# kevin-robb/live_ekf_slam

Measured on AMD Instinct MI355X. Metric: EKF predict-update steps/sec @ L=50, batch=65536; fp64 state RMSE vs ref, higher is better.
Workload: dtype f64

## Files before the change

live_ekf_slam_amd/csrc/capi_state.cpp:

```cpp
#include <stdio.h>
#include <string.h>

#include <vector>

#include "slam_handle.h"
#include "ekf_kernel.h"
#include "ukf_kernel.h"

using namespace slam_capi;

extern "C" {

int slam_get_sigma_points(slam_handle* h, int inst, double* X, int32_t* rows, int32_t* cols) {
    if (!h || inst < 0 || inst >= h->B) return slam_internal_fail(SLAM_ERR_ARG, "bad instance");
    TRY(flush_lazy(h));
    if (h->kind == SLAM_EKF_SLAM) return slam_internal_fail(SLAM_ERR_UNSUPPORTED, "sigma points exist for the UKF kinds only");
    if (!h->inited) return slam_internal_fail(SLAM_ERR_STATE, "slam_init has not been called");
    HIP_TRY(hipSetDevice(h->device));
    HIP_TRY(hipStreamSynchronize(h->stream));
    int32_t n = 0;
    HIP_TRY(hipMemcpy(&n, h->ukf.dnsq + inst, sizeof(int32_t), hipMemcpyDeviceToHost));
    n = n < 0 ? 0 : (n > h->n_max ? h->n_max : n);
    if (rows) *rows = n;
    if (cols) *cols = n > 0 ? 2 * n + 1 : 0;
// ... 201 lines not shown
    }
    std::vector<char> buf((size_t)64 << 20);
    for (const CkptItem& it : ckpt_items(h))
        for (size_t off = 0; off < it.bytes; off += buf.size()) {
            const size_t nb = it.bytes - off < buf.size() ? it.bytes - off : buf.size();
            if (fread(buf.data(), 1, nb, f) != nb) { fclose(f); return slam_internal_fail(SLAM_ERR_IO, "%s is truncated", path); }
            if (hipMemcpy((char*)it.dev + off, buf.data(), nb, hipMemcpyHostToDevice) != hipSuccess) { fclose(f); return slam_internal_fail(SLAM_ERR_HIP, "copying the state to the device failed"); }
        }
    fclose(f);
    h->step = hd.step; h->inited = hd.inited != 0; h->seed = hd.seed; h->inst0 = hd.inst0;
    h->ukf.predicted = false;
    TRY(map_track_reset(h));
    if (h->shadow) {
        const int tr = h->tracked;
        const int rc = slam_track_instance(h, tr);
        if (rc) return rc;
    }
    return SLAM_OK;
}

int slam_track_instance(slam_handle* h, int inst) {
    if (!h || inst >= h->B) return slam_internal_fail(SLAM_ERR_ARG, "bad instance");
    TRY(flush_lazy(h));
    if (h->ukf.predicted) return slam_internal_fail(SLAM_ERR_STATE, "a prediction stage is pending: call slam_update_dev first");
    if (h->shadow) { slam_destroy(h->shadow); h->shadow = nullptr; h->tracked = -1; }
    if (inst < 0) return SLAM_OK;
    if (h->kind != SLAM_EKF_SLAM) return slam_internal_fail(SLAM_ERR_UNSUPPORTED, "EKF handles only: the UKF launches every step at the call, there is no queue a getter would have to run");
    HIP_TRY(hipSetDevice(h->device));
    HIP_TRY(hipStreamSynchronize(h->stream));
    slam_handle* s = nullptr;
    int rc = slam_create(&h->cfg, h->kind, 1, h->L_max, h->dtype, h->device, &s);
    if (rc) return rc;
    s->lazy_max = 0;
    s->seed = h->seed; s->inst0 = h->inst0 + inst;
    s->range_max = h->range_max; s->fov_min = h->fov_min; s->fov_max = h->fov_max;
    s->waves_per_filter = h->waves_per_filter;
    if (!h->hmap.empty()) rc = slam_set_map(s, h->hmap.data(), (int)(h->hmap.size() / 2));
    if (!rc && h->each.maps_each)
        rc = slam_set_maps(s, h->each.hmaps.data() + (size_t)inst * h->each.map_stride * 2, h->each.hLs.data() + inst, h->each.map_stride);
    if (!rc && h->each.noise_each) rc = slam_set_noise_each(s, h->each.hnoise.data() + inst);
    if (!rc && h->inited) {
        const size_t b = (size_t)inst, e = (size_t)h->esz;
        hipError_t errs[] = {
            hipMemcpy(s->dP, (const char*)h->dP + b * h->pstride * e, (size_t)h->pstride * e, hipMemcpyDeviceToDevice),
            hipMemcpy(s->dx, (const char*)h->dx + b * h->xstride * e, (size_t)h->xstride * e, hipMemcpyDeviceToDevice),
            hipMemcpy(s->dM, h->dM + b, sizeof(int32_t), hipMemcpyDeviceToDevice),
            hipMemcpy(s->dids, h->dids + b * h->L_max, sizeof(int32_t) * h->L_max, hipMemcpyDeviceToDevice),
            hipMemcpy(s->dflags, h->dflags + b, sizeof(int32_t), hipMemcpyDeviceToDevice),
            hipMemcpy(s->dts, h->dts + b, sizeof(int32_t), hipMemcpyDeviceToDevice),
            hipMemcpy(s->dtruth, h->dtruth + 3 * b, sizeof(double) * 3, hipMemcpyDeviceToDevice),
            hipMemcpy(s->derr, h->derr + b, sizeof(double), hipMemcpyDeviceToDevice),
            h->ukf.dsq ? hipMemcpy(s->ukf.dsq, h->ukf.dsq + b * h->pstride, sizeof(double) * h->pstride, hipMemcpyDeviceToDevice) : hipSuccess,
            h->ukf.dnsq ? hipMemcpy(s->ukf.dnsq, h->ukf.dnsq + b, sizeof(int32_t), hipMemcpyDeviceToDevice) : hipSuccess,
            h->ukf.dxprev ? hipMemcpy(s->ukf.dxprev, h->ukf.dxprev + b * h->xstride, sizeof(double) * h->xstride, hipMemcpyDeviceToDevice) : hipSuccess,
            h->ukf.dvt ? hipMemcpy(s->ukf.dvt, h->ukf.dvt + b * h->pstride, sizeof(double) * h->pstride, hipMemcpyDeviceToDevice) : hipSuccess,
            h->ukf.dvage ? hipMemcpy(s->ukf.dvage, h->ukf.dvage + b, sizeof(int32_t), hipMemcpyDeviceToDevice) : hipSuccess,
        };
        for (hipError_t ee : errs)
            if (ee != hipSuccess) { slam_destroy(s); return slam_internal_fail(SLAM_ERR_HIP, "copying the tracked instance -> %s", hipGetErrorString(ee)); }
        s->step = h->step; s->inited = true;
    }
    if (rc) { slam_destroy(s); return rc; }
    h->shadow = s; h->tracked = inst;
    return SLAM_OK;
}

int slam_sync(slam_handle* h) {
    if (!h) return slam_internal_fail(SLAM_ERR_ARG, "NULL handle");
    TRY(flush_lazy(h));
    HIP_TRY(hipSetDevice(h->device));
    HIP_TRY(hipStreamSynchronize(h->stream));
    h->eager_target = h->eager_init;
    return SLAM_OK;
}
int slam_batch(const slam_handle* h) { return h ? h->B : 0; }
int slam_state_dim_max(const slam_handle* h) { return h ? h->n_max : 0; }

int slam_set_debug_flags(slam_handle* h, int flags) {
    if (!h) return slam_internal_fail(SLAM_ERR_ARG, "NULL handle");
    TRY(flush_lazy(h));
    HIP_TRY(hipSetDevice(h->device));
    HIP_TRY(hipStreamSynchronize(h->stream));
#ifndef SLAM_ABLATE
    flags &= (4 | 32 | 128);
#endif
    if ((flags & (4 | 32)) && !h->dprof) {
        HIP_TRY(h->dprof.reserve(slam::kEkfProfSlots * (size_t)h->B));
        HIP_TRY(hipMemset(h->dprof, 0, sizeof(unsigned long long) * h->dprof.cap()));
    }
    h->dbg = flags;
    return SLAM_OK;
}

int slam_variant_available(int L_max, int dtype, int variant) { return slam::ekf_variant_available(L_max, dtype == SLAM_F32, variant); }

int slam_k_histogram(slam_handle* h, uint64_t out[8], int reset) {
    if (!h || !out) return slam_internal_fail(SLAM_ERR_ARG, "bad argument");
    TRY(flush_lazy(h));
    HIP_TRY(hipSetDevice(h->device));
    HIP_TRY(h->kind == SLAM_EKF_SLAM ? hipStreamSynchronize(h->stream) : hipDeviceSynchronize());
    static_assert(sizeof(unsigned long long) == sizeof(uint64_t), "histogram element size");
    HIP_TRY(hipMemcpy(out, h->dkhist, sizeof(uint64_t) * 8, hipMemcpyDeviceToHost));
    if (reset) HIP_TRY(hipMemset(h->dkhist, 0, sizeof(uint64_t) * 8));
    return SLAM_OK;
}

int slam_traffic_counters(slam_handle* h, uint64_t out[4], int reset) {
    if (!h || !out) return slam_internal_fail(SLAM_ERR_ARG, "bad argument");
    if (h->kind != SLAM_EKF_SLAM) return slam_internal_fail(SLAM_ERR_UNSUPPORTED, "the traffic counters are kept by the EKF step kernels");
    TRY(flush_lazy(h));
    HIP_TRY(hipSetDevice(h->device));
    HIP_TRY(hipStreamSynchronize(h->stream));
    HIP_TRY(hipMemcpy(out, h->dkhist + slam::kEkfTrafficSlot, sizeof(uint64_t) * 4, hipMemcpyDeviceToHost));
    if (reset) HIP_TRY(hipMemset(h->dkhist + slam::kEkfTrafficSlot, 0, sizeof(uint64_t) * 4));
    return SLAM_OK;
}

int slam_reset_counters_async(slam_handle* h) {
    if (!h) return slam_internal_fail(SLAM_ERR_ARG, "bad argument");
    TRY(flush_lazy(h));
    HIP_TRY(hipSetDevice(h->device));
    HIP_TRY(hipMemsetAsync(h->dkhist, 0, sizeof(unsigned long long) * 16, h->stream));
    return SLAM_OK;
}

int slam_kernel_info(slam_handle* h, int multi_step, char* name, int name_cap, int32_t out[5]) {
    if (!h || (!name && !out)) return slam_internal_fail(SLAM_ERR_ARG, "bad argument");
    if (h->kind != SLAM_EKF_SLAM) return slam_internal_fail(SLAM_ERR_UNSUPPORTED, "EKF handles only");
    HIP_TRY(hipSetDevice(h->device));
    slam::EkfKernelInfo ki;
    HIP_TRY(slam::ekf_kernel_info(h->L_max, h->B, h->waves_per_filter, h->esz == 4, multi_step ? 1 : 0, &ki));
    if (name && name_cap > 0) { strncpy(name, ki.name, (size_t)name_cap - 1); name[name_cap - 1] = 0; }
    if (out) {
        hipDeviceProp_t pr;
        HIP_TRY(hipGetDeviceProperties(&pr, h->device));
        out[0] = ki.lds_bytes; out[1] = ki.vgprs; out[2] = ki.threads; out[3] = ki.wg_per_cu; out[4] = pr.multiProcessorCount;
    }
    return SLAM_OK;
}

int slam_ukf_sweep_stats(slam_handle* h, uint64_t out[2], int reset) {
    if (!h || !out) return slam_internal_fail(SLAM_ERR_ARG, "bad argument");
    if (h->kind == SLAM_EKF_SLAM) return slam_internal_fail(SLAM_ERR_STATE, "UKF handles only");
    TRY(flush_lazy(h));
    HIP_TRY(hipSetDevice(h->device));
    HIP_TRY(hipDeviceSynchronize());
    HIP_TRY(hipMemcpy(out, h->dkhist + 8, sizeof(uint64_t) * 2, hipMemcpyDeviceToHost));
    if (reset) HIP_TRY(hipMemset(h->dkhist + 8, 0, sizeof(uint64_t) * 2));
    return SLAM_OK;
}

int slam_ukf_set_sqrt_mode(slam_handle* h, int mode) {
    if (!h) return slam_internal_fail(SLAM_ERR_ARG, "bad argument");
    if (h->kind == SLAM_EKF_SLAM) return slam_internal_fail(SLAM_ERR_ARG, "the square-root mode is a UKF setting");
    if (mode != SLAM_UKF_SQRT_EIGEN && mode != SLAM_UKF_SQRT_CHOLESKY) return slam_internal_fail(SLAM_ERR_ARG, "unknown square-root mode %d", mode);
    if (mode == SLAM_UKF_SQRT_CHOLESKY && h->L_max > slam::kUkfLdsMaxLandmarks)
        return slam_internal_fail(SLAM_ERR_UNSUPPORTED, "the Cholesky square root exists for the LDS size classes only (L_max <= %d), this handle has L_max %d",
                                  slam::kUkfLdsMaxLandmarks, h->L_max);
    TRY(flush_lazy(h));
    HIP_TRY(hipSetDevice(h->device));
    if (mode == SLAM_UKF_SQRT_CHOLESKY) HIP_TRY(h->ukf.dchol.reserve((size_t)h->B));
    h->ukf.chol = mode == SLAM_UKF_SQRT_CHOLESKY;
    return SLAM_OK;
}

int slam_ukf_sqrt_stats(slam_handle* h, uint64_t out[2], int reset) {
    if (!h || !out) return slam_internal_fail(SLAM_ERR_ARG, "bad argument");
// ... 63 lines not shown
```

live_ekf_slam_amd/csrc/ekf_kernel_impl.h:

```cpp
#pragma once
#include "ekf_kernel.h"

#include <stdio.h>

#include <type_traits>

#include "../../include/slam_batch.h"
#include "ekf_model.h"
#include "slam_rng.h"
#include "sim_device.h"

namespace slam {

template <int NMAX, int W, int KG_, int UNR_, int KP_ = 0>
struct EkfGeom {
    static constexpr int TPB = 64 * W;
    static constexpr int LDP = (NMAX + 2) & ~1;
    static constexpr int LMAX = (NMAX - 3) / 2;
    static constexpr int KCAP = LMAX > 0 ? LMAX : 1;
    static constexpr int KG = KG_;
    static constexpr int KP = KP_ > 0 ? KP_ : ((KG_ > 5 && NMAX > 43 && W < 5) ? 3 : (KG_ > 4 ? 4 : KG_));
    static constexpr int KLOOP = 2 * KP;
    static constexpr int TS = 3 + 2 * KP;
    static constexpr int UNR = UNR_;
// ... 32 lines not shown
#endif
#ifndef SLAM_CTRL_ILP
#define SLAM_CTRL_ILP 1
#endif
#ifndef SLAM_CTRL_SG
#define SLAM_CTRL_SG 3
#endif
#ifndef SLAM_PRIO_THIN
#define SLAM_PRIO_THIN 2
#endif

#define SLAM_STAMP(i)                                                                    \
    do {                                                                                 \
        if (prof_on && tid == 0) {                                                       \
            const unsigned long long now_ = __builtin_readcyclecounter();                \
            p.prof[(size_t)blockIdx.x * kEkfProfSlots + (i)] += now_ - tprev;                            \
            tprev = now_;                                                                \
        }                                                                                \
    } while (0)

typedef double dbl2_t __attribute__((ext_vector_type(2)));
typedef float flt4_t __attribute__((ext_vector_type(4)));
template <class ST> struct Vec16;
template <> struct Vec16<double> {
    static constexpr int VEC = 2;
    typedef dbl2_t type;
};
template <> struct Vec16<float> {
    static constexpr int VEC = 4;
    typedef flt4_t type;
};

__device__ __forceinline__ int opaque(int v) {
    asm volatile("" : "+v"(v));
    return v;
}

typedef const __attribute__((address_space(4))) EkfStepParams* EkfColdParams;
__device__ __forceinline__ EkfColdParams ekf_cold_params() {
    EkfColdParams k = (EkfColdParams)__builtin_amdgcn_kernarg_segment_ptr();
    asm volatile("" : "+s"(k));
    return k;
}
struct EkfSimCold {
    uint64_t seed;
    int64_t inst0;
    double d_max, th_max, range_max, fov_min, fov_max;
};
struct EkfMapCold {
    const double* map;
    const double* map_each;
    const int32_t* L_each;
    int32_t map_stride, L;
};
struct EkfSimNoiseCold {
    double sV00, sV11, sW00, sW11;
    const NoiseRow* noise_each;
    int32_t sim;
};

__device__ __forceinline__ double rdlane(double v, int l) {
    const int lo = __builtin_amdgcn_readlane(__double2loint(v), l);
    const int hi = __builtin_amdgcn_readlane(__double2hiint(v), l);
    return __hiloint2double(hi, lo);
}

__device__ __forceinline__ unsigned hi_abs(double v) {
    return (unsigned)(__double_as_longlong(v) >> 32) & 0x7fffffffu;
}

template <int NMAX, int W, int KG_, int UNR_, class ST, int PIPE, bool MULTI, int KP_ = 0>
__global__ __launch_bounds__(64 * W, (W >= 2 ? 4 : SLAM_W1_WAVES)) void ekf_step_kernel(const EkfStepParams p) {
    using G = EkfGeom<NMAX, W, KG_, UNR_, KP_>;
    constexpr int TPB = G::TPB, LDP = G::LDP, KCAP = G::KCAP, LMAX = G::LMAX, KG = G::KG, KP = G::KP, KLOOP = G::KLOOP, TS = G::TS, UNR = G::UNR;

    __shared__ double s_xt[LDP];
    __shared__ double s_xp[LDP];
    __shared__ double s_R[TS * LDP];
    __shared__ double s_C[TS * LDP];
    __shared__ double2 s_K[KG * LDP];
    constexpr int VEC = Vec16<ST>::VEC;
    constexpr int HS = hp_substride<VEC>(LDP), HPW = (VEC - 1) * HS + (LDP + VEC - 1) / VEC;
    __shared__ double2 s_HP[KG * HPW];
    __shared__ double s_sc[16];
    constexpr int SD = SLAM_SD;
    __shared__ float s_meas[SD * 3 * KCAP];
    __shared__ double s_tru[SD * 6];
    __shared__ int s_kraw[SD];
    __shared__ int s_sim[2];
    __shared__ int s_ids[LMAX > 0 ? LMAX : 1];
    __shared__ int s_didx[2 * KCAP];
    __shared__ int s_next[2 * 4];
    __shared__ double s_ps[2 * 10];
    __shared__ int s_chunk;
    __shared__ int s_T[TS];
    __shared__ signed char s_slot[LDP];
    __shared__ signed char s_need[TS];
    __shared__ int s_misc[8];
    __shared__ double s_keep[4];
    __shared__ int s_kh[8];
    __shared__ int s_ring[8];
    __shared__ int s_pass[4];
    __shared__ int s_wend[KG];
    __shared__ unsigned s_cnt[4];

    const int b = blockIdx.x;
    const int tid = threadIdx.x;
    const int lane = tid & 63;
    const FilterNoise nz = filter_noise(p, b);
    if (p.long_mode == 1) {
        const int kk = p.meas_count_in[b];
        if ((kk < p.k_stride_in ? kk : p.k_stride_in) > p.long_cap) return;
    }

    const bool dump_meas = p.meas_out != nullptr;
    const bool prof_on = (p.dbg & 4) && p.prof != nullptr;
    unsigned long long tprev = prof_on ? __builtin_readcyclecounter() : 0ull;
    if (prof_on && tid < 64) p.prof[(size_t)blockIdx.x * kEkfProfSlots + tid] = 0ull;
    typedef typename Vec16<ST>::type VT;
    constexpr int ESZ = (int)sizeof(ST);
    auto hpi = [](int c) -> int { return (c & (VEC - 1)) * HS + (c / VEC); };
    const int T = MULTI ? p.T : 1;
    ST* const PA = const_cast<ST*>(static_cast<const ST*>(p.P)) + (size_t)b * p.pstride;
    ST* const PB = static_cast<ST*>(p.P_out) + (size_t)b * p.pstride;
    ST* const Pfinal = PA;
    ST* Pcur = PA;
    ST* __restrict__ xb = static_cast<ST*>(p.x) + (size_t)b * p.xstride;
    constexpr bool kWide = sizeof(ST) == 8;
    int flags = p.flags[b];
    const int M_init = p.M[b];
    double xpre[(LDP + TPB - 1) / TPB];
#pragma unroll
    for (int u = 0; u < (LDP + TPB - 1) / TPB; ++u) {
        const int i = tid + TPB * u;
        xpre[u] = (i < p.xstride && i < LDP) ? (double)xb[i] : 0.0;
    }
    const int idpre = (tid < p.L_max) ? p.ids[(size_t)b * p.L_max + tid] : 0;
    double keep0 = 0.0;
    if (p.sim && tid < 64) {
        if (tid < 3) keep0 = p.truth[3 * (size_t)b + tid];
        if (tid == 3) keep0 = p.err_sum[b];
    }
    const int n_init = 3 + 2 * M_init;
    const int ts0 = p.timestep[b];

    if (flags & SLAM_INST_INDEX_OOR) {
        return;
    }

#pragma unroll
    for (int u = 0; u < (LDP + TPB - 1) / TPB; ++u) {
        const int i = tid + TPB * u;
        if (i < LDP) {
            const double v = i < n_init ? xpre[u] : 0.0;
            s_xt[i] = v;
            s_xp[i] = v;
        }
    }
    if (tid < M_init) s_ids[tid] = idpre;
    if (tid < 4) s_keep[tid] = keep0;
#pragma unroll 1
    for (int i = tid; i < LDP; i += TPB) s_slot[i] = (signed char)(i < 3 ? i : -1);
    if (tid < TS) {
        s_T[tid] = tid < 3 ? tid : -1;
        s_need[tid] = (signed char)(tid < 3 ? 1 : 0);
    }
    if (tid < 8) s_kh[tid] = 0;
// ... 159 lines not shown
```

live_ekf_slam_amd/csrc/ekf_step_control.h:

```cpp

    auto leader_chain = [&](int ii, int si, float r_m, float b_m, double (&H)[8], double& nu0, double& nu1, double (&Si)[4]) -> bool {
        const double* const xl = p.lm_from_pred ? s_xp : s_xt;
        const double dx = xl[ii] - s_xp[0], dy = xl[ii + 1] - s_xp[1];
        const float dist = (float)sqrt(dx * dx + dy * dy);
        const double dd = (double)dist, d2 = (double)(dist * dist);
        const int hl = lane & 7;
        const bool usey = (hl == 1) || (hl == 3) || (hl == 4) || (hl == 6);
        const bool neg = (hl == 0) || (hl == 1) || (hl == 5) || (hl == 6);
        double num = usey ? dy : dx;
        num = neg ? -num : num;
        const double q = num / (hl < 4 ? dd : d2);
        const float angf = (float)rem2pi(det_atan2(dy, dx) - s_xp[2]);
        const float nu0f = r_m - dist - nz.w_r;
        const float nu1f = b_m - angf - nz.w_b;
        nu0 = (double)nu0f; nu1 = (double)nu1f;
#pragma unroll
        for (int j = 0; j < 8; ++j) H[j] = rdlane(q, j);
        const double h00 = H[0], h01 = H[1], h03 = H[2], h04 = H[3], h10 = H[4], h11 = H[5], h12 = -1.0, h13 = H[6], h14 = H[7];
        const int cs = lane < 3 ? lane : (lane == 3 ? ii : ii + 1);
        const double p0 = s_R[cs], p1 = s_R[LDP + cs], p2 = s_R[2 * LDP + cs], pi = s_R[si * LDP + cs], pj = s_R[(si + 1) * LDP + cs];
        const double gx = ((h00 * p0 + h01 * p1) + h03 * pi) + h04 * pj;
        const double gy = (((h10 * p0 + h11 * p1) + h12 * p2) + h13 * pi) + h14 * pj;
        const double g0x = rdlane(gx, 0), g1x = rdlane(gx, 1), g2x = rdlane(gx, 2), gix = rdlane(gx, 3), gjx = rdlane(gx, 4);
        const double g0y = rdlane(gy, 0), g1y = rdlane(gy, 1), g2y = rdlane(gy, 2), giy = rdlane(gy, 3), gjy = rdlane(gy, 4);
// ... 6 lines not shown
        S[3] = S[3] + nz.W11;
        return inv2x2_lu(S, Si);
    };

    auto form_known = [&](const int* didx_g, int k, int l0, int lim, int nsrc, int& l1_out, int& nT_out) -> int {
        const int l1 = (k - l0 < lim) ? k : l0 + lim;
        const int ng = l1 - l0;
        const int idx = (lane < ng) ? didx_g[l0 + lane] : -1;
        const int myii = idx >= 0 ? 3 + 2 * idx : -1;
        const int cur = (lane < KP) ? s_T[3 + 2 * lane] : -1;
        bool dupl = false, has = false, keep = false;
#pragma unroll
        for (int w = 0; w < KP; ++w) {
            const int ii_w = __builtin_amdgcn_readlane(myii, w), cur_w = __builtin_amdgcn_readlane(cur, w);
            dupl = dupl || (w < lane && ii_w == myii);
            has = has || (cur_w >= 0 && cur_w == myii);
            keep = keep || (ii_w >= 0 && ii_w == cur);
        }
        const bool wantv = myii >= 0 && !dupl;
        const bool release = lane < KP && cur >= 0 && !keep;
        if (release) {
            s_slot[cur] = (signed char)-1; s_slot[cur + 1] = (signed char)-1;
            s_T[3 + 2 * lane] = -1; s_T[4 + 2 * lane] = -1;
        }
        const bool freeslot = lane < KP && (cur < 0 || !keep);
        const unsigned long long fmask = __ballot(freeslot);
        const bool needs = wantv && !has;
        const unsigned long long nmask = __ballot(needs);
        const int rank = __popcll(nmask & ((1ull << lane) - 1ull));
        int j = 0;
        {
            unsigned long long fm = fmask;
#pragma unroll
            for (int w = 0; w < KP; ++w) {
                const int lowest = __ffsll((long long)fm) - 1;
                if (w == rank) j = lowest;
                fm &= fm - 1ull;
            }
        }
        bool gath = false;
        if (needs) {
            s_T[3 + 2 * j] = myii; s_T[4 + 2 * j] = myii + 1;
            s_slot[myii] = (signed char)(3 + 2 * j); s_slot[myii + 1] = (signed char)(4 + 2 * j);
            const signed char nd = (signed char)(myii < nsrc ? 1 : 2);
            s_need[3 + 2 * j] = nd; s_need[4 + 2 * j] = nd;
            gath = nd == 1;
        }
        unsigned long long occ = __ballot(lane < KP && cur >= 0 && keep);
        {
            unsigned long long fm = fmask;
            const int ntake = __popcll(nmask);
#pragma unroll
            for (int w = 0; w < KP; ++w) {
                const int lowest = __ffsll((long long)fm) - 1;
                if (w < ntake && lowest >= 0) occ |= 1ull << lowest;
                fm &= fm - 1ull;
            }
        }
        l1_out = l1;
        nT_out = occ ? 5 + 2 * (63 - __clzll((long long)occ)) : 3;
        return __ballot(gath) != 0ull ? 1 : 0;
    };

    auto thin_downdate = [&](int j0, int jstride, int s0, int sstride, int nTd, int nd, const double2* __restrict__ Ku,
                             const double2* __restrict__ HPu) {
        const int* const Ttab = s_T;
#pragma unroll 1
        for (int j = j0; j < nd; j += jstride) {
            const double2 kj = Ku[j], hj = HPu[hpi(j)];
#pragma unroll 2
            for (int sl = s0; sl < nTd; sl += sstride) {
                const int t_s = Ttab[sl];
                if ((unsigned)t_s < (unsigned)nd) {
                    const double2 kt = Ku[t_s], ht = HPu[hpi(t_s)];
                    const int i = sl * LDP + j;
                    s_R[i] = ekf_downdate(s_R[i], kt.x, kt.y, hj.x, hj.y);
                    s_C[i] = ekf_downdate(s_C[i], kj.x, kj.y, ht.x, ht.y);
                }
            }
        }
    };

    constexpr int NU = (LDP + 63) / 64;
    auto thin_downdate_ctl = [&](int nTd, int nd, const double2* __restrict__ Ku, const double2* __restrict__ HPu, const double2 (&kj)[NU],
                                 const double2 (&hj)[NU]) {
        constexpr int SG = SLAM_CTRL_SG;
        int tsv[TS];
#pragma unroll
        for (int sl = 0; sl < TS; ++sl) tsv[sl] = s_T[sl];
#pragma unroll
        for (int s0 = 0; s0 < TS; s0 += SG) {
            if (s0 >= nTd) break;
            double2 kt[SG], ht[SG];
            double rv[SG][NU], cv[SG][NU];
            bool ok[SG];
#pragma unroll
            for (int g = 0; g < SG; ++g) {
                const int sl = s0 + g < TS ? s0 + g : TS - 1;
                const int t_s = tsv[sl];
                ok[g] = s0 + g < nTd && (unsigned)t_s < (unsigned)nd;
                const int tc = ok[g] ? t_s : 0;
                kt[g] = Ku[tc]; ht[g] = HPu[hpi(tc)];
#pragma unroll
                for (int u = 0; u < NU; ++u) {
                    const int j = lane + 64 * u;
                    const int i = sl * LDP + (j < LDP ? j : 0);
                    rv[g][u] = s_R[i]; cv[g][u] = s_C[i];
                }
            }
#pragma unroll
            for (int g = 0; g < SG; ++g) {
                if (!ok[g]) continue;
                const int sl = s0 + g;
#pragma unroll
                for (int u = 0; u < NU; ++u) {
                    const int j = lane + 64 * u;
                    if (j < nd) {
                        const int i = sl * LDP + j;
                        s_R[i] = ekf_downdate(rv[g][u], kt[g].x, kt[g].y, hj[u].x, hj[u].y);
                        s_C[i] = ekf_downdate(cv[g][u], kj[u].x, kj[u].y, ht[g].x, ht[g].y);
                    }
                }
            }
        }
    };
```

live_ekf_slam_amd/csrc/ekf_step_decoupled.h:

```cpp

    if constexpr (MULTI && W >= 2) {
        auto fastable = [&](int tq) -> bool {
            const int* nx = s_next + 4 * (tq & 1);
            constexpr int kStepMax = sizeof(ST) == 8 ? KLOOP : (KLOOP < KG ? KLOOP : KG);
            return nx[0] <= kStepMax && nx[1] == 0 && nx[2] == 0 && nx[3] == 0;
        };
        const bool fast_ok = p.id_known && !dump_meas && fastable(t) &&
                             !SLAM_DBG(p.dbg & (2 | 16 | 64));
        if (fast_ok) {
            const int n = na, ldn = ekf_ld(n, ESZ);
            ST* const Pbuf = Pcur;
            constexpr int kFirstStreamer = 1;
            constexpr int NS = W - kFirstStreamer;
            constexpr bool kGen = W >= 2;
            if (tid == 0) {
                s_ring[0] = nu; s_ring[1] = 0; s_ring[2] = 0; s_ring[3] = 0; s_ring[4] = t; s_ring[5] = 0; s_ring[6] = 0; s_ring[7] = 0;
                s_pass[0] = 0; s_pass[1] = 0; s_pass[2] = 0; s_pass[3] = 0;
            }
            __syncthreads();
            auto ld_i = [](int* q) -> int { return __hip_atomic_load(q, __ATOMIC_RELAXED, __HIP_MEMORY_SCOPE_WORKGROUP); };
            auto st_i = [](int* q, int v) { __hip_atomic_store(q, v, __ATOMIC_RELAXED, __HIP_MEMORY_SCOPE_WORKGROUP); };
            constexpr int kSpinBudget = 1 << 21;
            auto spin_over = [&](int& spins) -> bool {
                spins += 1;
// ... 84 lines not shown
                                        }
                                    }
                                }
#pragma unroll
                                for (int g = 0; g < GB; ++g)
                                    if (g < nb) {
                                        s_R[ss[g] * LDP + j] = j < n ? rv[g] : 0.0;
                                        s_C[ss[g] * LDP + j] = j < n ? cv[g] : 0.0;
                                    }
                            }
#pragma unroll
                            for (int g = 0; g < GB; ++g)
                                if (g < nb && ss[g] >= 3 && lane < 3) {
                                    s_R[ss[g] * LDP + lane] = s_C[lane * LDP + ts[g]];
                                    s_C[ss[g] * LDP + lane] = s_R[lane * LDP + ts[g]];
                                }
                        }
                        if (lane == 0) st_i(&s_ring[6], 0);
                    }
                    if (lane < TS) s_need[lane] = 0;
                    SLAM_STAMP(18);
                    if (l0q == 0) {
                        const double* const ps = s_ps + 10 * pq;
                        const double* const r2o = s_R + 2 * LDP;
                        const double* const c2o = s_C + 2 * LDP;
                        const double fa = ps[3], fb = ps[4];
                        const double p22 = r2o[2];
                        auto predicted = [&](double tv, int r, int cc) -> double {
                            const double f_r = r == 0 ? fa : fb;
                            if (r < 2) tv = tv + f_r * r2o[cc];
                            if (cc < 2) {
                                double a2 = c2o[r];
                                if (r < 2) a2 = a2 + f_r * p22;
                                tv = tv + a2 * (cc == 0 ? fa : fb);
                            }
                            if (r < 2 && cc < 2) tv = tv + ps[5 + 2 * r + cc];
                            if (r == 2 && cc == 2) tv = tv + nz.V11;
                            return tv;
                        };
                        double n_r0 = 0.0, n_r1 = 0.0, n_c0 = 0.0, n_c1 = 0.0, n_22 = 0.0;
                        const int t_s = (lane >= 2 && lane < nTq) ? s_T[lane] : -1;
                        const bool thin_l = (unsigned)t_s < (unsigned)n;
                        if (thin_l) {
                            n_r0 = predicted(s_R[lane * LDP + 0], t_s, 0);
                            n_r1 = predicted(s_R[lane * LDP + 1], t_s, 1);
                            n_c0 = predicted(s_C[lane * LDP + 0], 0, t_s);
                            n_c1 = predicted(s_C[lane * LDP + 1], 1, t_s);
                            if (lane == 2) n_22 = predicted(p22, 2, 2);
                        }
#pragma unroll
                        for (int u = 0; u < (LDP + 63) / 64; ++u) {
                            const int j = lane + 64 * u;
                            if (j >= 2 && j < n) {
                                const double r2 = r2o[j], c2 = c2o[j];
                                s_R[j] = ekf_pred_row(s_R[j], fa, r2);
                                s_R[LDP + j] = ekf_pred_row(s_R[LDP + j], fb, r2);
                                s_C[j] = ekf_pred_col(s_C[j], c2, fa);
                                s_C[LDP + j] = ekf_pred_col(s_C[LDP + j], c2, fb);
                            }
                        }
                        if (lane < 2) {
                            const int j = lane;
                            const double v00 = predicted(s_R[j], 0, j), v10 = predicted(s_R[LDP + j], 1, j);
                            const double w00 = predicted(s_C[j], j, 0), w10 = predicted(s_C[LDP + j], j, 1);
                            s_R[j] = v00; s_R[LDP + j] = v10; s_C[j] = w00; s_C[LDP + j] = w10;
                        }
                        if (thin_l) {
                            s_R[lane * LDP + 0] = n_r0; s_R[lane * LDP + 1] = n_r1;
                            s_C[lane * LDP + 0] = n_c0; s_C[lane * LDP + 1] = n_c1;
                            if (lane == 2) { s_R[2 * LDP + 2] = n_22; s_C[2 * LDP + 2] = n_22; }
                        }
                    }
                    SLAM_STAMP(19);
#pragma unroll 1
                    for (int l = l0q; l < l1q; ++l) {
                        const int idx = didx_q[l];
                        if (idx < 0) continue;
                        const float r_m = meas_q[3 * l + 1], b_m = meas_q[3 * l + 2];
                        const int ii = 3 + 2 * idx;
                        const int si = s_slot[ii];
                        double H[8], Si[4], nu0, nu1;
                        if (!leader_chain(ii, si, r_m, b_m, H, nu0, nu1, Si)) fl_or |= SLAM_INST_S_SINGULAR;
                        SLAM_STAMP(20);
                        for (int sp = 0; pub - ld_i(&s_ring[1]) >= KG && !spin_over(sp);) __builtin_amdgcn_s_sleep(SLAM_SLEEP_RING);
                        if (ld_i(&s_ring[2])) break;
                        SLAM_STAMP(21);
                        const int slot = pub % KG;
                        double2* __restrict__ HPu = s_HP + slot * HPW;
                        double2* __restrict__ Ku = s_K + slot * LDP;
                        double2 kreg[NU], hreg[NU];
#pragma unroll
                        for (int u = 0; u < NU; ++u) { kreg[u] = make_double2(0.0, 0.0); hreg[u] = make_double2(0.0, 0.0); }
                        if (!SLAM_DBG(p.dbg & 512)) {
                            const double h00 = H[0], h01 = H[1], h03 = H[2], h04 = H[3], h10 = H[4], h11 = H[5], h12 = -1.0, h13 = H[6], h14 = H[7];
                            const double* Ri = s_R + si * LDP;
                            const double* Rj = s_R + (si + 1) * LDP;
                            const double* Ci = s_C + si * LDP;
                            const double* Cj = s_C + (si + 1) * LDP;
#pragma unroll
                            for (int u = 0; u < (LDP + 63) / 64; ++u) {
                                const int c = lane + 64 * u;
                                double2 hp = make_double2(0.0, 0.0), kk = make_double2(0.0, 0.0);
                                if (c < n) {
                                    const double p0 = s_R[c], p1 = s_R[LDP + c], p2 = s_R[2 * LDP + c], pi = Ri[c], pj = Rj[c];
                                    hp.x = ((h00 * p0 + h01 * p1) + h03 * pi) + h04 * pj;
                                    hp.y = (((h10 * p0 + h11 * p1) + h12 * p2) + h13 * pi) + h14 * pj;
                                    const double q0 = s_C[c], q1 = s_C[LDP + c], q2 = s_C[2 * LDP + c], qi = Ci[c], qj = Cj[c];
                                    const double phx = ((q0 * h00 + q1 * h01) + qi * h03) + qj * h04;
                                    const double phy = (((q0 * h10 + q1 * h11) + q2 * h12) + qi * h13) + qj * h14;
                                    kk.x = phx * Si[0] + phy * Si[2];
                                    kk.y = phx * Si[1] + phy * Si[3];
                                    double xv = s_xp[c] + (kk.x * nu0 + kk.y * nu1);
                                    if (c == 2) xv = rem2pi(xv);
                                    s_xp[c] = xv;
                                }
                                if (c < LDP) { HPu[hpi(c)] = hp; Ku[c] = kk; }
                                kreg[u] = kk; hreg[u] = hp;
                            }
                        }
                        if (!kWide && lane == 0) s_wend[slot] = (l == lastu) ? 1 : 0;
                        __builtin_amdgcn_fence(__ATOMIC_RELEASE, "workgroup");
                        pub += 1;
                        if (lane == 0) st_i(&s_ring[0], pub);
                        SLAM_STAMP(22);
                        if (!SLAM_DBG(p.dbg & 256)) {
#if SLAM_CTRL_ILP
                            thin_downdate_ctl(nTq, n, Ku, HPu, kreg, hreg);
#else
                            thin_downdate(lane, 64, 0, 1, nTq, n, Ku, HPu);
#endif
                        }
                    }
                    l0q = l1q;
                    } while (l0q < kq && !ld_i(&s_ring[2]));
                    if (ld_i(&s_ring[2])) break;
                    SLAM_STAMP(23);
                    if (p.sim && lane == 0) {
                        const double* tru = s_tru + (tt % SD) * 6 + 3;
                        const double ex = (double)(float)s_xp[0] - tru[0], ey = (double)(float)s_xp[1] - tru[1];
                        s_keep[3] = s_keep[3] + sqrt(ex * ex + ey * ey);
                    }
#pragma unroll 1
                    for (int i = lane; i < n; i += 64) {
                        const ST sv = (ST)s_xp[i];
                        s_xt[i] = (double)sv;
                        s_xp[i] = (double)sv;
                        const unsigned h0 = hi_abs((double)sv);
                        hiacc = hiacc > h0 ? hiacc : h0;
                    }
                    if constexpr (!kWide) {
                        const int nel = nTq * LDP;
#pragma unroll 1
                        for (int i0 = lane; i0 < nel; i0 += 256) {
                            double rv[4], cv[4];
#pragma unroll
                            for (int u = 0; u < 4; ++u) {
                                const int i = i0 + 64 * u < nel ? i0 + 64 * u : i0;
                                rv[u] = s_R[i]; cv[u] = s_C[i];
                            }
#pragma unroll
                            for (int u = 0; u < 4; ++u) {
                                const int i = i0 + 64 * u;
                                if (i < nel) { s_R[i] = (double)(ST)rv[u]; s_C[i] = (double)(ST)cv[u]; }
                            }
                        }
                    }
                    if ((p.dbg & 32) && p.prof != nullptr && lane == 0 && tt < kEkfProfSlots)
                        p.prof[(size_t)blockIdx.x * kEkfProfSlots + tt] = (wall_clock64() << 4) | (unsigned long long)(kq < 15 ? kq : 15);
                    tt += 1;
                    SLAM_STAMP(24);
                    if (tt >= T) break;
                    if constexpr (kGen) {
                        for (int sp = 0; ld_i(&s_sim[0]) <= tt && !spin_over(sp);) __builtin_amdgcn_s_sleep(1);
                        __builtin_amdgcn_fence(__ATOMIC_ACQUIRE, "workgroup");
                    }
                    SLAM_STAMP(26);
                    prestep(tt);
                    SLAM_STAMP(25);
                    if (!fastable(tt)) break;
                }
                if (lane == 0) {
                    s_ring[4] = tt;
                    s_ring[5] = fl_or;
                    __builtin_amdgcn_fence(__ATOMIC_RELEASE, "workgroup");
                    st_i(&s_ring[3], 1);
                    if (ld_i(&s_ring[2])) st_i(&s_ring[6], 0);
                }
                __builtin_amdgcn_s_setprio(0);
            }
            if (is_streamer) {
                __builtin_amdgcn_s_setprio(0);
                const bool leader = (tid >> 6) == kFirstStreamer;
#ifdef SLAM_PASS_MIN_FORCE
                constexpr int kPassMinCfg = SLAM_PASS_MIN_FORCE;
#else
#ifdef SLAM_PASS_MIN_F32
                constexpr int kPassMinF32 = SLAM_PASS_MIN_F32;
#else
                constexpr int kPassMinF32 = KG > 4 ? KG - 2 : 3;
#endif
                constexpr int kPassMinCfg = kWide ? (KG > SLAM_PASS_MIN + 1 ? KG - 1 : SLAM_PASS_MIN) : kPassMinF32;
#endif
                constexpr int kPassMin = kPassMinCfg < KG ? kPassMinCfg : KG;
                int seen = 0;
                int sp = 0;
#pragma unroll 1
                for (;;) {
                    if (leader) {
                        int app, pend;
                        bool stop = false;
#pragma unroll 1
                        for (;;) {
                            if (spin_over(sp)) { stop = true; break; }
// ... 96 lines not shown
```

live_ekf_slam_amd/csrc/ekf_step_prestep.h:

```cpp

    auto finish = [&](int steps_done, int Mf, int fl, bool pre) {
        const EkfColdParams pc = ekf_cold_params();
        const int nfin = 3 + 2 * Mf;
        for (int i = tid; i < nfin; i += TPB) xb[i] = (ST)s_xt[i];
        if (Mf != M_init) {
            int32_t* const ids_b = pc->ids + (size_t)b * pc->L_max;
            for (int i = tid; i < Mf; i += TPB) ids_b[i] = s_ids[i];
        }
        const bool simf = pc->sim != 0;
        if (tid == 0) {
            pc->M[b] = Mf;
            pc->flags[b] = fl;
            pc->timestep[b] = ts0 + steps_done;
            if (simf) pc->err_sum[b] = s_keep[3];
        }
        if (simf && tid < 3) {
            const int tq = pre ? steps_done : steps_done - 1;
            pc->truth[3 * (size_t)b + tid] = steps_done == 0 && !pre ? s_keep[tid] : s_tru[(tq % SD) * 6 + (pre ? 0 : 3) + tid];
        }
        unsigned long long* const kh = pc->khist;
        if (kh != nullptr && tid < 8 && s_kh[tid] != 0) atomicAdd(&kh[tid], (unsigned long long)s_kh[tid]);
        if (kh != nullptr && tid >= 8 && tid < 12) {
            const unsigned long long v = s_cnt[tid - 8] + (tid == 9 ? (unsigned long long)((nfin + 8) * ESZ / 8) : 0ull);
            const unsigned long long unit = tid == 8 ? 16ull : (tid == 9 ? 8ull : 1ull);
            if (v != 0ull) atomicAdd(&kh[kEkfTrafficSlot + tid - 8], v * unit);
        }
    };

    int M = M_init;
    int na = n_init;
    int nu = 0;
    unsigned hiacc = 0u;

    auto simgen = [&](int tn) {
        const int sq = tn % SD;
        const EkfColdParams pc = ekf_cold_params();
        if (!p.sim) {
            const int ksi = pc->k_stride_in;
            const size_t row = (size_t)tn * pc->B + b;
            int kk = pc->meas_count_in[row];
            kk = kk < ksi ? kk : ksi;
            kk = kk < 0 ? 0 : kk;
            const int kc = kk < KCAP ? kk : KCAP;
            const float* src = pc->meas_in + row * ksi * 3;
            for (int i = lane; i < 3 * kc; i += 64) s_meas[sq * 3 * KCAP + i] = src[i];
            if (lane == 0) s_kraw[sq] = kk;
            return;
        }
        const float* const cp = p.cmd_each ? p.cmd_each + ((size_t)tn * p.B + b) * 2 : (MULTI ? p.cmds + 2 * tn : nullptr);
        const float fwd_n = (MULTI || cp) ? cp[0] : p.fwd;
        const float ang_n = (MULTI || cp) ? cp[1] : p.ang;
        double tx = s_keep[0], ty = s_keep[1], tth = s_keep[2];
        if (lane == 0) { s_tru[sq * 6 + 0] = tx; s_tru[sq * 6 + 1] = ty; s_tru[sq * 6 + 2] = tth; }
        const EkfSimCold sc = {pc->seed, pc->inst0, pc->d_max, pc->th_max, pc->range_max, pc->fov_min, pc->fov_max};
        const EkfMapCold mc = {pc->map, pc->map_each, pc->L_each, pc->map_stride, pc->L};
        const EkfSimNoiseCold nc = {pc->sV00, pc->sV11, pc->sW00, pc->sW11, pc->noise_each, 1};
        const int Lm = sim_map_size(mc, b);
        const double* const map = sim_map(mc, b);
        const double lmx0 = lane < Lm ? map[2 * lane] : 0.0, lmy0 = lane < Lm ? map[2 * lane + 1] : 0.0;
        const int kr = sim_wave<KCAP, false>(sc, b, lane, fwd_n, ang_n, pc->step + (uint32_t)tn, map, Lm, tx, ty, tth, lmx0, lmy0,
                                             s_meas + sq * 3 * KCAP, sim_noise(nc, b));
        if (lane == 0) {
            s_keep[0] = tx; s_keep[1] = ty; s_keep[2] = tth;
            s_tru[sq * 6 + 3] = tx; s_tru[sq * 6 + 4] = ty; s_tru[sq * 6 + 5] = tth;
            s_kraw[sq] = kr;
        }
    };
    auto prestep = [&](int tn) {
        const double* const xv = s_xp;
        const int qb = tn & 1;
        float* meas = s_meas + (tn % SD) * 3 * KCAP;
        int* didx = s_didx + qb * KCAP;
        int* nx = s_next + 4 * qb;
        double* ps = s_ps + 10 * qb;
        const float* const cp = p.cmd_each ? p.cmd_each + ((size_t)tn * p.B + b) * 2 : (MULTI ? p.cmds + 2 * tn : nullptr);
        const float fwd_n = (MULTI || cp) ? cp[0] : p.fwd;
        const float ang_n = (MULTI || cp) ? cp[1] : p.ang;
        if (s_sim[0] <= tn) {
            simgen(tn);
            if (lane == 0) s_sim[0] = tn + 1;
        }
        __builtin_amdgcn_fence(__ATOMIC_SEQ_CST, "wavefront");
        const int kraw = s_kraw[tn % SD];
        {
            const double x0 = (double)(ST)xv[0], x1 = (double)(ST)xv[1], th = (double)(ST)xv[2];
            double sn, cs;
            det_sincos(th, &sn, &cs);
            const float dd = fwd_n + nz.v_d;
            const double cv = cs * nz.V00, sv = sn * nz.V00;
            if (lane == 0) {
                nx[0] = kraw;
                ps[0] = x0 + (double)dd * cs;
                ps[1] = x1 + (double)dd * sn;
                ps[2] = rem2pi((th + (double)ang_n) + (double)nz.v_th);
                ps[3] = (double)(-1 * fwd_n) * sn;
                ps[4] = (double)fwd_n * cs;
                ps[5] = cv * cs; ps[6] = cv * sn; ps[7] = sv * cs; ps[8] = sv * sn;
            }
        }
#ifdef SLAM_EXP_ASSOC_REP
#pragma unroll 1
        for (int rep_ = 0; rep_ <= SLAM_EXP_ASSOC_REP; ++rep_)
#endif
        if (p.id_known) {
            const int kn = kraw < KCAP ? kraw : KCAP;
            const int room = (p.L_max < LMAX ? p.L_max : LMAX) - M;
            int nins = 0;
            bool frz = false, capf = false;
            if (kn <= 64 && M <= 64) {
                const int myid = lane < kn ? (int)meas[3 * lane] : -1;
                const int sid = lane < M ? s_ids[lane] : 0;
                int idx = -1, firstl = lane;
                bool isnew = false;
#pragma unroll 1
                for (int l = 0; l < kn; ++l) {
                    const int id = __builtin_amdgcn_readlane(myid, l);
                    const unsigned long long m = __ballot(lane < M && sid == id);
                    const unsigned long long e = __ballot(lane < l && myid == id);
                    if (lane == l) { idx = m ? __ffsll((long long)m) - 1 : -1; isnew = m == 0ull; firstl = e ? __ffsll((long long)e) - 1 : l; }
                }
                const bool isfirst = isnew && firstl == lane;
                const unsigned long long fmask = __ballot(isfirst);
                const int rankf = __popcll(fmask & ((1ull << firstl) - 1ull));
                const bool insf = rankf < room;
                const unsigned long long fz = __ballot(isnew && !isfirst && insf);
                const unsigned long long cm = __ballot(isnew && !insf);
                const unsigned long long before = fz ? ((1ull << (__ffsll((long long)fz) - 1)) - 1ull) : ~0ull;
                frz = fz != 0ull;
                capf = (cm & before) != 0ull;
                if (isnew) idx = (isfirst && insf) ? M + rankf : -1;
                if (lane < kn) didx[lane] = idx;
                nins = __popcll(fmask);
                nins = nins < room ? nins : (room > 0 ? room : 0);
            } else {
                int nfirst = 0;
#pragma unroll 1
                for (int l = 0; l < kn && !frz; ++l) {
                    const int id = (int)meas[3 * l];
                    int found = -1;
#pragma unroll 1
                    for (int j0 = 0; j0 < M && found < 0; j0 += 64) {
                        const int j = j0 + lane;
                        const unsigned long long m = __ballot(j < M && s_ids[j] == id);
                        if (m != 0ull) found = j0 + (__ffsll((long long)m) - 1);
                    }
                    int code = found;
                    if (found < 0) {
                        int first = -1;
#pragma unroll 1
                        for (int q0 = 0; q0 < l && first < 0; q0 += 64) {
                            const int q = q0 + lane;
                            const unsigned long long m = __ballot(q < l && (int)meas[3 * (q < l ? q : 0)] == id);
                            if (m != 0ull) first = q0 + (__ffsll((long long)m) - 1);
                        }
                        if (first < 0) {
                            code = nfirst < room ? M + nfirst : -1;
                            capf = capf || nfirst >= room;
                            nfirst += 1;
                        } else if (didx[first] >= M) {
                            frz = true;
                        } else {
                            code = -1;
                            capf = true;
                        }
                    }
                    if (lane == 0) didx[l] = code;
                    __builtin_amdgcn_fence(__ATOMIC_SEQ_CST, "wavefront");
                }
                nins = nfirst < room ? nfirst : (room > 0 ? room : 0);
            }
            if (lane == 0) {
                nx[3] = capf ? 1 : 0;
                nx[1] = nins;
                nx[2] = frz ? 1 : 0;
            }
        }
    };
// ... 1 lines not shown
```

Baseline: 72.33 million.

## Decouple leader thin downdate from ring-slot publish using private scratch buffers

The leader wave now writes its K and HP rows for the touched slots into a private shared scratch area (s_sc, enlarged) and runs its thin downdate from there. When no ring slot is free it defers publishing to the follower ring until after the downdate, so it no longer stalls before doing its own work. The downdate also reads the slot list through a single ballot instead of a per-slot register array. A debug flag (1024) forces the deferred path, and the shared-memory footprint grows slightly, which could lower occupancy.

```diff
diff --git a/live_ekf_slam_amd/csrc/capi_state.cpp b/live_ekf_slam_amd/csrc/capi_state.cpp
--- a/live_ekf_slam_amd/csrc/capi_state.cpp
+++ b/live_ekf_slam_amd/csrc/capi_state.cpp
@@ -307,7 +307,7 @@
     HIP_TRY(hipSetDevice(h->device));
     HIP_TRY(hipStreamSynchronize(h->stream));
 #ifndef SLAM_ABLATE
-    flags &= (4 | 32 | 128);
+    flags &= (4 | 32 | 128 | 1024);
 #endif
     if ((flags & (4 | 32)) && !h->dprof) {
         HIP_TRY(h->dprof.reserve(slam::kEkfProfSlots * (size_t)h->B));
diff --git a/live_ekf_slam_amd/csrc/ekf_kernel_impl.h b/live_ekf_slam_amd/csrc/ekf_kernel_impl.h
--- a/live_ekf_slam_amd/csrc/ekf_kernel_impl.h
+++ b/live_ekf_slam_amd/csrc/ekf_kernel_impl.h
@@ -138,7 +138,8 @@
     constexpr int VEC = Vec16<ST>::VEC;
     constexpr int HS = hp_substride<VEC>(LDP), HPW = (VEC - 1) * HS + (LDP + VEC - 1) / VEC;
     __shared__ double2 s_HP[KG * HPW];
-    __shared__ double s_sc[16];
+    constexpr int kScN = (MULTI && W >= 2 && 4 * TS > 16) ? 4 * TS : 16;
+    __shared__ __attribute__((aligned(16))) double s_sc[kScN];
     constexpr int SD = SLAM_SD;
     __shared__ float s_meas[SD * 3 * KCAP];
     __shared__ double s_tru[SD * 6];
diff --git a/live_ekf_slam_amd/csrc/ekf_step_control.h b/live_ekf_slam_amd/csrc/ekf_step_control.h
--- a/live_ekf_slam_amd/csrc/ekf_step_control.h
+++ b/live_ekf_slam_amd/csrc/ekf_step_control.h
@@ -112,12 +112,11 @@
     };
 
     constexpr int NU = (LDP + 63) / 64;
-    auto thin_downdate_ctl = [&](int nTd, int nd, const double2* __restrict__ Ku, const double2* __restrict__ HPu, const double2 (&kj)[NU],
+    auto thin_downdate_ctl = [&](int nTd, int nd, const double2* __restrict__ Kt, const double2* __restrict__ Ht, const double2 (&kj)[NU],
                                  const double2 (&hj)[NU]) {
         constexpr int SG = SLAM_CTRL_SG;
-        int tsv[TS];
-#pragma unroll
-        for (int sl = 0; sl < TS; ++sl) tsv[sl] = s_T[sl];
+        const int t_l = lane < nTd ? s_T[lane] : -1;
+        const unsigned okm = (unsigned)__ballot((unsigned)t_l < (unsigned)nd);
 #pragma unroll
         for (int s0 = 0; s0 < TS; s0 += SG) {
             if (s0 >= nTd) break;
@@ -127,10 +126,8 @@
 #pragma unroll
             for (int g = 0; g < SG; ++g) {
                 const int sl = s0 + g < TS ? s0 + g : TS - 1;
-                const int t_s = tsv[sl];
-                ok[g] = s0 + g < nTd && (unsigned)t_s < (unsigned)nd;
-                const int tc = ok[g] ? t_s : 0;
-                kt[g] = Ku[tc]; ht[g] = HPu[hpi(tc)];
+                ok[g] = ((okm >> (s0 + g)) & 1u) != 0u;
+                kt[g] = Kt[sl]; ht[g] = Ht[sl];
 #pragma unroll
                 for (int u = 0; u < NU; ++u) {
                     const int j = lane + 64 * u;
diff --git a/live_ekf_slam_amd/csrc/ekf_step_decoupled.h b/live_ekf_slam_amd/csrc/ekf_step_decoupled.h
--- a/live_ekf_slam_amd/csrc/ekf_step_decoupled.h
+++ b/live_ekf_slam_amd/csrc/ekf_step_decoupled.h
@@ -190,12 +190,13 @@
                         double H[8], Si[4], nu0, nu1;
                         if (!leader_chain(ii, si, r_m, b_m, H, nu0, nu1, Si)) fl_or |= SLAM_INST_S_SINGULAR;
                         SLAM_STAMP(20);
+#if !SLAM_CTRL_ILP
                         for (int sp = 0; pub - ld_i(&s_ring[1]) >= KG && !spin_over(sp);) __builtin_amdgcn_s_sleep(SLAM_SLEEP_RING);
                         if (ld_i(&s_ring[2])) break;
                         SLAM_STAMP(21);
-                        const int slot = pub % KG;
-                        double2* __restrict__ HPu = s_HP + slot * HPW;
-                        double2* __restrict__ Ku = s_K + slot * LDP;
+#endif
+                        double2* const s_kt = reinterpret_cast<double2*>(s_sc);
+                        double2* const s_ht = s_kt + TS;
                         double2 kreg[NU], hreg[NU];
 #pragma unroll
                         for (int u = 0; u < NU; ++u) { kreg[u] = make_double2(0.0, 0.0); hreg[u] = make_double2(0.0, 0.0); }
@@ -222,21 +223,50 @@
                                     if (c == 2) xv = rem2pi(xv);
                                     s_xp[c] = xv;
                                 }
-                                if (c < LDP) { HPu[hpi(c)] = hp; Ku[c] = kk; }
                                 kreg[u] = kk; hreg[u] = hp;
                             }
-                        }
-                        if (!kWide && lane == 0) s_wend[slot] = (l == lastu) ? 1 : 0;
-                        __builtin_amdgcn_fence(__ATOMIC_RELEASE, "workgroup");
-                        pub += 1;
-                        if (lane == 0) st_i(&s_ring[0], pub);
+#pragma unroll
+                            for (int u = 0; u < NU; ++u) {
+                                const int c = lane + 64 * u;
+                                const int sc = c < n ? (int)s_slot[c] : -1;
+                                if (sc >= 0) { s_kt[sc] = kreg[u]; s_ht[sc] = hreg[u]; }
+                            }
+                        }
+                        auto publish = [&]() {
+                            const int slot = pub % KG;
+                            double2* __restrict__ HPu = s_HP + slot * HPW;
+                            double2* __restrict__ Ku = s_K + slot * LDP;
+#pragma unroll
+                            for (int u = 0; u < NU; ++u) {
+                                const int c = lane + 64 * u;
+                                if (c < LDP) { HPu[hpi(c)] = hreg[u]; Ku[c] = kreg[u]; }
+                            }
+                            if (!kWide && lane == 0) s_wend[slot] = (l == lastu) ? 1 : 0;
+                            __builtin_amdgcn_fence(__ATOMIC_RELEASE, "workgroup");
+                            pub += 1;
+                            if (lane == 0) st_i(&s_ring[0], pub);
+                        };
+#if SLAM_CTRL_ILP
+                        const bool slot_free = __builtin_amdgcn_readfirstlane(pub - ld_i(&s_ring[1])) < KG && !(p.dbg & 1024);
+#else
+                        constexpr bool slot_free = true;
+#endif
+                        if (slot_free) publish();
                         SLAM_STAMP(22);
                         if (!SLAM_DBG(p.dbg & 256)) {
 #if SLAM_CTRL_ILP
-                            thin_downdate_ctl(nTq, n, Ku, HPu, kreg, hreg);
+                            thin_downdate_ctl(nTq, n, s_kt, s_ht, kreg, hreg);
 #else
-                            thin_downdate(lane, 64, 0, 1, nTq, n, Ku, HPu);
+                            thin_downdate(lane, 64, 0, 1, nTq, n, s_K + ((pub - 1) % KG) * LDP, s_HP + ((pub - 1) % KG) * HPW);
 #endif
+                        }
+                        if (!slot_free) {
+                            SLAM_STAMP(23);
+                            for (int sp = 0; pub - ld_i(&s_ring[1]) >= KG && !spin_over(sp);) __builtin_amdgcn_s_sleep(SLAM_SLEEP_RING);
+                            if (ld_i(&s_ring[2])) break;
+                            SLAM_STAMP(21);
+                            publish();
+                            SLAM_STAMP(22);
                         }
                     }
                     l0q = l1q;
diff --git a/live_ekf_slam_amd/csrc/ekf_step_prestep.h b/live_ekf_slam_amd/csrc/ekf_step_prestep.h
--- a/live_ekf_slam_amd/csrc/ekf_step_prestep.h
+++ b/live_ekf_slam_amd/csrc/ekf_step_prestep.h
@@ -88,11 +88,14 @@
             det_sincos(th, &sn, &cs);
             const float dd = fwd_n + nz.v_d;
             const double cv = cs * nz.V00, sv = sn * nz.V00;
+            int v_th_bits = __float_as_int(nz.v_th);
+            if constexpr (MULTI) asm volatile("" : "+s"(v_th_bits));
+            const float v_th = __int_as_float(v_th_bits);
             if (lane == 0) {
                 nx[0] = kraw;
                 ps[0] = x0 + (double)dd * cs;
                 ps[1] = x1 + (double)dd * sn;
-                ps[2] = rem2pi((th + (double)ang_n) + (double)nz.v_th);
+                ps[2] = rem2pi((th + (double)ang_n) + (double)v_th);
                 ps[3] = (double)(-1 * fwd_n) * sn;
                 ps[4] = (double)fwd_n * cs;
                 ps[5] = cv * cs; ps[6] = cv * sn; ps[7] = sv * cs; ps[8] = sv * sn;
```

Measured after the change: 73.72 million (median of 6 runs). +1.9%, better.
